# mokemokechicken/reversi-alpha-zero

Hardware: NVIDIA H100
Metric: self_play_games_per_sec (higher is better)
Workload: dtype f16

## Files before the change

reversi-alpha-zero_b200/csrc/rz_net_tc.cu:

```cuda
#include <stdlib.h>
#include <type_traits>
#include "rz_bitboard.cuh"
#include "rz_net.cuh"
#include "rz_tc_common.cuh"

namespace rz {
namespace tc {

constexpr uint32_t kProducerRegs = 40, kMathRegs = 232;
constexpr int kMathThreads = 256;
constexpr uint32_t kActCg = 2896, kActSlot = 144;
constexpr uint32_t kActBytes = 32 * kActCg;
constexpr uint32_t kStageBytes = 32768, kStages = 3;
constexpr int kResAhead = 4;
constexpr uint32_t kA0Bytes = 8192, kW0Bytes = 16384;
constexpr uint32_t kOffAct = 0;
constexpr uint32_t kOffW = kOffAct + kActBytes;
constexpr uint32_t kOffA0 = kOffW + kStages * kStageBytes;
constexpr uint32_t kOffW0 = kOffA0 + kA0Bytes;
constexpr uint32_t kOffSS = kOffW0 + kW0Bytes;
constexpr uint32_t kOffHw = kOffSS + 2 * 2048;
constexpr uint32_t kOffBar = kOffHw + 768 * 4;
constexpr uint32_t kNumBars = 2 * kStages + 1;
constexpr uint32_t kSmemBytes = kOffBar + kNumBars * 8;
constexpr uint32_t kSmemAlloc = kSmemBytes + 128;
static_assert(kSmemAlloc <= 232448, "shared memory budget exceeded");
static_assert(kTowerResFloatsPerCta == (size_t)kMathThreads * 128, "residual scratch per CTA");

#ifdef RZ_TOWER_STAMPS
enum : int {
    kStTiles,
    kStTile,
    kStKLoop,
    kStFull,
    kStMma,
    kStEpiBar,
    kStEpi0,
    kStEpi1,
    kStEpi2,
    kStEpiLast,
    kStFeat,
    kStEmpty,
    kStCount
};
constexpr int kStMaxCtas = 1024;
__device__ unsigned long long g_tower_stamps[kStMaxCtas][kStCount];
__device__ __forceinline__ void stamp_add(int phase, uint32_t cycles) { atomicAdd(&g_tower_stamps[blockIdx.x][phase], (unsigned long long)cycles); }
#define RZ_STAMP(...) __VA_ARGS__
#else
#define RZ_STAMP(...)
#endif

template <int CL>
__global__ void __launch_bounds__(kThreads, 1) net_tower_kernel(const Params pp) {
    Params p = pp;
    if (p.n_dev) p.n = *p.n_dev;
    extern __shared__ uint8_t smem_raw[];
    const uint32_t base = (smem_u32(smem_raw) + 127u) & ~127u;
    uint8_t* sm = smem_raw + (base - smem_u32(smem_raw));
    const int warp = threadIdx.x >> 5, lane = threadIdx.x & 31;
    const uint32_t bar0 = base + kOffBar;
    auto bar_full = [&](uint32_t s) { return bar0 + s * 8; };
    auto bar_empty = [&](uint32_t s) { return bar0 + (kStages + s) * 8; };
    const uint32_t bar_w0 = bar0 + 2 * kStages * 8;
    const uint32_t ntiles = (p.n + 1) >> 1;
    const int L = p.n_layers;
    const uint32_t crank = CL > 1 ? cluster_ctarank() : 0u;
    const uint32_t cbase = blockIdx.x - crank;
    const uint32_t iters = cbase < ntiles ? (ntiles - cbase + gridDim.x - 1) / gridDim.x : 0u;

    for (uint32_t i = threadIdx.x * 16; i < kActBytes; i += kThreads * 16) *reinterpret_cast<uint4*>(sm + kOffAct + i) = make_uint4(0, 0, 0, 0);
    fence_proxy_async();
    for (uint32_t i = threadIdx.x; i < 768; i += kThreads)
        reinterpret_cast<float*>(sm + kOffHw)[i] = __ldg(i < 512 ? p.blob + p.off_policy_conv + i : p.blob + p.off_value_conv + (i - 512));
    if (threadIdx.x == 0) {
        for (uint32_t s = 0; s < kStages; ++s) { mbar_init(bar_full(s), 1); mbar_init(bar_empty(s), 8 * CL); }
        mbar_init(bar_w0, 1);
        asm volatile("fence.mbarrier_init.release.cluster;" ::: "memory");
    }
    __syncthreads();
    if (CL > 1) cluster_sync_all();

    if (warp >= 8) {
        asm volatile("setmaxnreg.dec.sync.aligned.u32 %0;" ::"n"(kProducerRegs));
        if (warp == 8 && lane == 0) {
            if (iters > 0) {
                mbar_expect_tx(bar_w0, kW0Bytes);
                bulk_g2s(base + kOffW0, p.w0, kW0Bytes, bar_w0);
            }
            uint32_t stage = 0, phase = 0;
            for (uint32_t it = 0; it < iters; ++it) {
                for (int l = 1; l < L; ++l) {
                    const uint8_t* src = reinterpret_cast<const uint8_t*>(p.w) + (size_t)(l - 1) * 36 * kStageBytes;
                    RZ_STAMP(uint32_t st_empty = 0;)
                    for (int s = 0; s < 36; ++s) {
                        RZ_STAMP(const uint32_t c0 = (uint32_t)clock();)
                        mbar_wait(bar_empty(stage), phase ^ 1);
                        RZ_STAMP(st_empty += (uint32_t)clock() - c0;)
                        mbar_expect_tx(bar_full(stage), kStageBytes);
                        if (CL == 1) {
                            bulk_g2s(base + kOffW + stage * kStageBytes, src + (size_t)s * kStageBytes, kStageBytes, bar_full(stage));
                        } else {
                            constexpr uint32_t kSlice = kStageBytes / CL;
                            bulk_g2s_mc(base + kOffW + stage * kStageBytes + crank * kSlice, src + (size_t)s * kStageBytes + crank * kSlice,
                                        kSlice, bar_full(stage), (uint16_t)((1u << CL) - 1u));
                        }
                        if (++stage == kStages) { stage = 0; phase ^= 1; }
                    }
                    RZ_STAMP(stamp_add(kStEmpty, st_empty);)
                }
            }
        }
    } else {
        asm volatile("setmaxnreg.inc.sync.aligned.u32 %0;" ::"n"(kMathRegs));
        const int et = threadIdx.x;
        const int wg = warp >> 2;
        const int r0 = wg * 64 + (warp & 3) * 16 + (lane >> 2);
        const int g0 = r0 >> 3, x = r0 & 7, y = g0 >> 1;
        const int cq = 2 * (lane & 3);
        const uint32_t act_row0 = base + kOffAct + (g0 + 2) * kActSlot + (x + 1) * 16 + cq * 2;
        const uint32_t act_row1 = act_row0 + kActSlot;
        const uint32_t a_wg = base + kOffAct + wg * 8 * kActSlot;
        float* ss_s = reinterpret_cast<float*>(sm + kOffSS);
        float4* res = reinterpret_cast<float4*>(p.res + (size_t)blockIdx.x * kTowerResFloatsPerCta) + et;
        const float* hw = reinterpret_cast<const float*>(sm + kOffHw);
        uint32_t stage = 0, phase = 0, ss_buf = 0;
        float d[128];
        ss_s[et] = __ldg(p.ss + et);
        ss_s[256 + et] = __ldg(p.ss + 256 + et);

        for (uint32_t it = 0; it < iters; ++it) {
            const uint32_t tile = blockIdx.x + it * gridDim.x;
            const uint32_t pos0 = tile * 2;
            RZ_STAMP(const uint32_t st_tile0 = (uint32_t)clock();)
            {
                const int m = et & 127, g = m >> 3, brd = g & 1;
                const bool valid = pos0 + brd < p.n;
                build_layer0_operand(sm + kOffA0, valid ? p.own[pos0 + brd] : 0, valid ? p.enemy[pos0 + brd] : 0, 2 * (et >> 7), g, m & 7,
                                     g >> 1);
                fence_proxy_async();
            }
            float hs[6];
            for (int l = 0; l < L; ++l) {
                const float* sc = ss_s + ss_buf * 512;
                const bool is_conv2 = l > 0 && (l & 1) == 0;
                float4 rb[kResAhead];
                RZ_STAMP(uint32_t st_c = (uint32_t)clock(), st_bar = 0, st_full = 0, st_mma = 0;)
                epi_bar();
                RZ_STAMP(st_bar += (uint32_t)clock() - st_c;)
                {
                    const size_t nl = l + 1 < L ? (size_t)l + 1 : 0;
                    const uint32_t dst = smem_u32(ss_s + (ss_buf ^ 1) * 512 + et);
                    cp_async_4(dst, p.ss + nl * 512 + et);
                    cp_async_4(dst + 1024, p.ss + nl * 512 + 256 + et);
                }
                RZ_STAMP(const uint32_t st_k0 = (uint32_t)clock();)
                acc_fence(d);
                if (l == 0) {
                    RZ_STAMP(st_c = (uint32_t)clock();)
                    mbar_wait(bar_w0, 0);
                    RZ_STAMP(st_full += (uint32_t)clock() - st_c;)
                    wgmma_fence();
#pragma unroll
                    for (uint32_t j = 0; j < 2; ++j)
                        wgmma_m64n256k16(d, smem_desc(base + kOffA0 + j * 2 * 2048 + wg * 1024, 2048, 128),
                                         smem_desc(base + kOffW0 + j * 2 * 4096, 4096, 128), j);
                    wgmma_commit();
                    RZ_STAMP(st_c = (uint32_t)clock();)
                    wgmma_wait<0>();
                    RZ_STAMP(st_mma += (uint32_t)clock() - st_c;)
                } else {
                    int prev = -1;
                    for (uint32_t tap = 0; tap < 9; ++tap) {
                        const uint32_t a_tap = a_wg + (2 * (tap / 3)) * kActSlot + (tap % 3) * 16;
                        for (uint32_t kb = 0; kb < 4; ++kb) {
                            RZ_STAMP(st_c = (uint32_t)clock();)
                            mbar_wait(bar_full(stage), phase);
                            RZ_STAMP(st_full += (uint32_t)clock() - st_c;)
                            const uint32_t b_st = base + kOffW + stage * kStageBytes;
                            wgmma_fence();
#pragma unroll
                            for (uint32_t j = 0; j < 4; ++j)
                                wgmma_m64n256k16(d, smem_desc(a_tap + (kb * 8 + 2 * j) * kActCg, kActCg, kActSlot),
                                                 smem_desc(b_st + 2 * j * 4096, 4096, 128), (tap | kb | j) != 0);
                            wgmma_commit();
                            RZ_STAMP(st_c = (uint32_t)clock();)
                            wgmma_wait<1>();
                            RZ_STAMP(st_mma += (uint32_t)clock() - st_c;)
                            if (prev >= 0 && lane == 0) {
                                mbar_arrive(bar_empty(prev));
                                if (CL > 1) mbar_arrive_cta(bar_empty(prev), crank ^ 1u);
                            }
                            prev = (int)stage;
                            if (++stage == kStages) { stage = 0; phase ^= 1; }
                        }
                    }
                    if (is_conv2) {
#pragma unroll
                        for (int i = 0; i < kResAhead; ++i) rb[i] = res[i * 256];
                    }
                    RZ_STAMP(st_c = (uint32_t)clock();)
                    wgmma_wait<0>();
                    RZ_STAMP(st_mma += (uint32_t)clock() - st_c;)
                    if (lane == 0) {
                        mbar_arrive(bar_empty(prev));
                        if (CL > 1) mbar_arrive_cta(bar_empty(prev), crank ^ 1u);
                    }
                }
                RZ_STAMP(const uint32_t st_k1 = (uint32_t)clock();)
                acc_fence(d);
                cp_async_wait_all();
                ss_buf ^= 1;
                const bool keep_res = l == 0 || is_conv2;
                const bool last = l == L - 1;
                RZ_STAMP(st_c = (uint32_t)clock();)
                if (!last) epi_bar();
                RZ_STAMP(const uint32_t st_e0 = (uint32_t)clock(); st_bar += st_e0 - st_c;)
                float* dbg0 = nullptr;
                float* dbg1 = nullptr;
                if (last && p.dbg_tower) {
                    if (pos0 < p.n) dbg0 = p.dbg_tower + ((size_t)pos0 * 64 + y * 8 + x) * 256;
                    if (pos0 + 1 < p.n) dbg1 = p.dbg_tower + ((size_t)(pos0 + 1) * 64 + y * 8 + x) * 256;
                }
                constexpr int kEpiRelu = 0, kEpiKeep = 1, kEpiLast = 2;
                auto epilogue = [&](auto conv2, auto kind) {
                    constexpr bool kConv2 = decltype(conv2)::value;
                    constexpr bool kKeep = decltype(kind)::value == kEpiKeep, kLast = decltype(kind)::value == kEpiLast;
                    if (kLast) {
#pragma unroll
                        for (int k = 0; k < 6; ++k) hs[k] = 0.f;
                    }
#pragma unroll
                for (int i = 0; i < 32; ++i) {
                    const int c = 8 * i + cq;
                    const float2 s = *reinterpret_cast<const float2*>(sc + c);
                    const float2 b = *reinterpret_cast<const float2*>(sc + 256 + c);
                    float v0 = fmaf(d[4 * i + 0], s.x, b.x), v1 = fmaf(d[4 * i + 1], s.y, b.y);
                    float v2 = fmaf(d[4 * i + 2], s.x, b.x), v3 = fmaf(d[4 * i + 3], s.y, b.y);
                    if (kConv2) {
                        const float4 r = rb[i % kResAhead];
                        if (i + kResAhead < 32) rb[i % kResAhead] = res[(i + kResAhead) * 256];
                        v0 += r.x; v1 += r.y; v2 += r.z; v3 += r.w;
                    }
                    if (kKeep || kLast) {
                        v0 = fmaxf(v0, 0.f); v1 = fmaxf(v1, 0.f); v2 = fmaxf(v2, 0.f); v3 = fmaxf(v3, 0.f);
                    }
                    if (!kLast) {
                        if (kKeep) res[i * 256] = make_float4(v0, v1, v2, v3);
                        const uint32_t h0 = pack_h2<!kKeep>(v0, v1);
                        const uint32_t h1 = pack_h2<!kKeep>(v2, v3);
                        const uint32_t off = (c >> 3) * kActCg;
                        asm volatile("st.shared.b32 [%0], %1;" ::"r"(act_row0 + off), "r"(h0) : "memory");
                        asm volatile("st.shared.b32 [%0], %1;" ::"r"(act_row1 + off), "r"(h1) : "memory");
                    } else {
                        const float4 w = *reinterpret_cast<const float4*>(hw + 2 * c);
                        const float2 wv = *reinterpret_cast<const float2*>(hw + 512 + c);
                        hs[0] = fmaf(v1, w.z, fmaf(v0, w.x, hs[0]));
                        hs[1] = fmaf(v1, w.w, fmaf(v0, w.y, hs[1]));
                        hs[2] = fmaf(v1, wv.y, fmaf(v0, wv.x, hs[2]));
                        hs[3] = fmaf(v3, w.z, fmaf(v2, w.x, hs[3]));
                        hs[4] = fmaf(v3, w.w, fmaf(v2, w.y, hs[4]));
                        hs[5] = fmaf(v3, wv.y, fmaf(v2, wv.x, hs[5]));
                        if (dbg0) *reinterpret_cast<float2*>(dbg0 + c) = make_float2(v0, v1);
                        if (dbg1) *reinterpret_cast<float2*>(dbg1 + c) = make_float2(v2, v3);
                    }
                }
                };
                using Conv2 = std::true_type;
                using NoConv2 = std::false_type;
                if (last) {
                    if (is_conv2) epilogue(Conv2(), std::integral_constant<int, kEpiLast>());
                    else epilogue(NoConv2(), std::integral_constant<int, kEpiLast>());
                } else if (is_conv2) {
                    epilogue(Conv2(), std::integral_constant<int, kEpiKeep>());
                } else if (keep_res) {
                    epilogue(NoConv2(), std::integral_constant<int, kEpiKeep>());
                } else {
                    epilogue(NoConv2(), std::integral_constant<int, kEpiRelu>());
                }
                if (!last) fence_proxy_async();
                RZ_STAMP(if (et == 0) {
                    stamp_add(kStKLoop, st_k1 - st_k0); stamp_add(kStFull, st_full); stamp_add(kStMma, st_mma); stamp_add(kStEpiBar, st_bar);
                    stamp_add(l == 0 ? kStEpi0 : last ? kStEpiLast : is_conv2 ? kStEpi2 : kStEpi1, (uint32_t)clock() - st_e0);
                })
            }
            RZ_STAMP(const uint32_t st_h0 = (uint32_t)clock();)
#pragma unroll
            for (int k = 0; k < 6; ++k) {
                hs[k] += __shfl_xor_sync(0xffffffffu, hs[k], 1);
                hs[k] += __shfl_xor_sync(0xffffffffu, hs[k], 2);
            }
            {
                const int q = lane & 3;
                if (q < 2 && pos0 + q < p.n) {
                    const float h0 = q ? hs[3] : hs[0], h1 = q ? hs[4] : hs[1], h2 = q ? hs[5] : hs[2];
                    store_head_features(p.feat + (size_t)(pos0 + q) * kHeadFeatures, p.ss + (size_t)L * 512, y * 8 + x, h0 + 0.f,
                                        h1 + 0.f, h2 + 0.f);
                }
            }
            RZ_STAMP(if (et == 0) {
                const uint32_t st_h1 = (uint32_t)clock();
                stamp_add(kStFeat, st_h1 - st_h0); stamp_add(kStTile, st_h1 - st_tile0); stamp_add(kStTiles, 1);
            })
        }
    }

    __syncthreads();
    if (CL > 1) cluster_sync_all();
}

int launch_tower(const Params& p, cudaStream_t stream) {
    return launch_tower_pairs<net_tower_kernel<1>, net_tower_kernel<2>, kSmemAlloc, 2>(p, stream);
}

}

static int g_cluster = 0;

int set_tower_cluster(int cluster) {
    RZ_REQUIRE(cluster == 1 || cluster == 2, "rz_net_set_tower_cluster: cluster must be 1 or 2");
    g_cluster = cluster;
    return RZ_OK;
}

int tower_cluster() {
    if (g_cluster == 0) {
        const char* cs = getenv("RZ_TOWER_CLUSTER");
        g_cluster = (cs && atoi(cs) == 1) ? 1 : 2;
    }
    return g_cluster;
}

}

#ifdef RZ_TOWER_STAMPS
extern "C" int rz_tower_stamps(unsigned long long* out, int n_ctas, int reset) {
    using namespace rz::tc;
    if (n_ctas < 0 || n_ctas > kStMaxCtas) return (int)cudaErrorInvalidValue;
    const size_t bytes = (size_t)n_ctas * kStCount * sizeof(unsigned long long);
    cudaError_t e = cudaDeviceSynchronize();
    if (e == cudaSuccess && out) e = cudaMemcpyFromSymbol(out, g_tower_stamps, bytes);
    if (e == cudaSuccess && reset) {
        void* dev = nullptr;
        e = cudaGetSymbolAddress(&dev, g_tower_stamps);
        if (e == cudaSuccess) e = cudaMemset(dev, 0, sizeof(g_tower_stamps));
        if (e == cudaSuccess) e = cudaDeviceSynchronize();
    }
    return (int)e;
}
extern "C" int rz_tower_stamp_count() { return rz::tc::kStCount; }
#endif
```

reversi-alpha-zero_b200/csrc/rz_tc_common.cuh:

```cuda
#pragma once
#include <cuda_fp16.h>
#include "rz_bitboard.cuh"
#include "rz_net.cuh"

namespace rz {
namespace tc {

__device__ __forceinline__ uint32_t smem_u32(const void* p) { return (uint32_t)__cvta_generic_to_shared(p); }

__device__ __forceinline__ void mbar_init(uint32_t bar, uint32_t count) {
    asm volatile("mbarrier.init.shared::cta.b64 [%0], %1;" ::"r"(bar), "r"(count) : "memory");
}
__device__ __forceinline__ void mbar_expect_tx(uint32_t bar, uint32_t bytes) {
    asm volatile("mbarrier.arrive.expect_tx.shared::cta.b64 _, [%0], %1;" ::"r"(bar), "r"(bytes) : "memory");
}
__device__ __forceinline__ void mbar_arrive(uint32_t bar) {
    asm volatile("mbarrier.arrive.shared::cta.b64 _, [%0];" ::"r"(bar) : "memory");
}
__device__ __forceinline__ void mbar_arrive_cta(uint32_t bar, uint32_t rank) {
    uint32_t remote;
    asm volatile("mapa.shared::cluster.u32 %0, %1, %2;" : "=r"(remote) : "r"(bar), "r"(rank));
    asm volatile("mbarrier.arrive.shared::cluster.b64 _, [%0];" ::"r"(remote) : "memory");
}
__device__ __forceinline__ void mbar_wait(uint32_t bar, uint32_t parity) {
    uint32_t ok = 0;
    long long t0 = 0;
    for (uint32_t spin = 0; !ok; ++spin) {
        asm volatile(
            "{\n\t.reg .pred p;\n\t"
            "mbarrier.try_wait.parity.shared::cta.b64 p, [%1], %2;\n\t"
            "selp.u32 %0, 1, 0, p;\n\t}"
            : "=r"(ok)
            : "r"(bar), "r"(parity)
            : "memory");
        if (!ok && (spin & 1023) == 1023) {
            const long long now = clock64();
            if (t0 == 0) t0 = now;
            else if (now - t0 > 8000000000LL) __trap();
        }
    }
}
__device__ __forceinline__ void bulk_g2s(uint32_t dst, const void* src, uint32_t bytes, uint32_t bar) {
    asm volatile("cp.async.bulk.shared::cluster.global.mbarrier::complete_tx::bytes [%0], [%1], %2, [%3];" ::"r"(dst), "l"(src),
                 "r"(bytes), "r"(bar)
                 : "memory");
}
__device__ __forceinline__ void bulk_g2s_mc(uint32_t dst, const void* src, uint32_t bytes, uint32_t bar, uint16_t mask) {
    asm volatile(
        "cp.async.bulk.shared::cluster.global.mbarrier::complete_tx::bytes.multicast::cluster [%0], [%1], %2, [%3], %4;" ::"r"(dst),
        "l"(src), "r"(bytes), "r"(bar), "h"(mask)
        : "memory");
}
__device__ __forceinline__ void cluster_sync_all() {
    asm volatile("barrier.cluster.arrive.release.aligned;\n\tbarrier.cluster.wait.acquire.aligned;" ::: "memory");
}
__device__ __forceinline__ uint32_t cluster_ctarank() {
    uint32_t r;
    asm volatile("mov.u32 %0, %%cluster_ctarank;" : "=r"(r));
    return r;
}
__device__ __forceinline__ void cp_async_4(uint32_t dst, const void* src) {
    asm volatile("cp.async.ca.shared.global [%0], [%1], 4;" ::"r"(dst), "l"(src) : "memory");
}
__device__ __forceinline__ void cp_async_wait_all() { asm volatile("cp.async.wait_all;" ::: "memory"); }
__device__ __forceinline__ void fence_proxy_async() { asm volatile("fence.proxy.async.shared::cta;" ::: "memory"); }
__device__ __forceinline__ void epi_bar() { asm volatile("bar.sync 1, 256;" ::: "memory"); }

__device__ __forceinline__ uint64_t smem_desc(uint32_t addr, uint32_t lbo, uint32_t sbo) {
    return (uint64_t)((addr >> 4) & 0x3FFF) | ((uint64_t)((lbo >> 4) & 0x3FFF) << 16) | ((uint64_t)((sbo >> 4) & 0x3FFF) << 32);
}
__device__ __forceinline__ void wgmma_fence() { asm volatile("wgmma.fence.sync.aligned;" ::: "memory"); }
__device__ __forceinline__ void wgmma_commit() { asm volatile("wgmma.commit_group.sync.aligned;" ::: "memory"); }
template <int N>
__device__ __forceinline__ void wgmma_wait() { asm volatile("wgmma.wait_group.sync.aligned %0;" ::"n"(N) : "memory"); }
__device__ __forceinline__ void acc_fence(float (&d)[128]) {
#pragma unroll
    for (int i = 0; i < 128; ++i) asm volatile("" : "+f"(d[i])::"memory");
}

#define RZ_D4(i) "+f"(d[i]), "+f"(d[i + 1]), "+f"(d[i + 2]), "+f"(d[i + 3])
#define RZ_D16(i) RZ_D4(i), RZ_D4(i + 4), RZ_D4(i + 8), RZ_D4(i + 12)
__device__ __forceinline__ void wgmma_m64n256k16(float (&d)[128], uint64_t adesc, uint64_t bdesc, uint32_t accumulate) {
    asm volatile(
        "{\n\t.reg .pred p;\n\t"
        "setp.ne.b32 p, %130, 0;\n\t"
        "wgmma.mma_async.sync.aligned.m64n256k16.f32.f16.f16 {"
        "%0, %1, %2, %3, %4, %5, %6, %7, %8, %9, %10, %11, %12, %13, %14, %15, "
        "%16, %17, %18, %19, %20, %21, %22, %23, %24, %25, %26, %27, %28, %29, %30, %31, "
        "%32, %33, %34, %35, %36, %37, %38, %39, %40, %41, %42, %43, %44, %45, %46, %47, "
        "%48, %49, %50, %51, %52, %53, %54, %55, %56, %57, %58, %59, %60, %61, %62, %63, "
        "%64, %65, %66, %67, %68, %69, %70, %71, %72, %73, %74, %75, %76, %77, %78, %79, "
        "%80, %81, %82, %83, %84, %85, %86, %87, %88, %89, %90, %91, %92, %93, %94, %95, "
        "%96, %97, %98, %99, %100, %101, %102, %103, %104, %105, %106, %107, %108, %109, %110, %111, "
        "%112, %113, %114, %115, %116, %117, %118, %119, %120, %121, %122, %123, %124, %125, %126, %127"
        "}, %128, %129, p, 1, 1, 0, 0;\n\t}"
        : RZ_D16(0), RZ_D16(16), RZ_D16(32), RZ_D16(48), RZ_D16(64), RZ_D16(80), RZ_D16(96), RZ_D16(112)
        : "l"(adesc), "l"(bdesc), "r"(accumulate)
        : "memory");
}
template <int O>
__device__ __forceinline__ void wgmma_m64n128k16(float (&d)[128], uint64_t adesc, uint64_t bdesc, uint32_t accumulate) {
    asm volatile(
        "{\n\t.reg .pred p;\n\t"
        "setp.ne.b32 p, %66, 0;\n\t"
        "wgmma.mma_async.sync.aligned.m64n128k16.f32.f16.f16 {"
        "%0, %1, %2, %3, %4, %5, %6, %7, %8, %9, %10, %11, %12, %13, %14, %15, "
        "%16, %17, %18, %19, %20, %21, %22, %23, %24, %25, %26, %27, %28, %29, %30, %31, "
        "%32, %33, %34, %35, %36, %37, %38, %39, %40, %41, %42, %43, %44, %45, %46, %47, "
        "%48, %49, %50, %51, %52, %53, %54, %55, %56, %57, %58, %59, %60, %61, %62, %63"
        "}, %64, %65, p, 1, 1, 0, 0;\n\t}"
        : RZ_D16(O), RZ_D16(O + 16), RZ_D16(O + 32), RZ_D16(O + 48)
        : "l"(adesc), "l"(bdesc), "r"(accumulate)
        : "memory");
}
template <int O>
__device__ __forceinline__ void wgmma_m64n64k16(float (&d)[128], uint64_t adesc, uint64_t bdesc, uint32_t accumulate) {
    asm volatile(
        "{\n\t.reg .pred p;\n\t"
        "setp.ne.b32 p, %34, 0;\n\t"
        "wgmma.mma_async.sync.aligned.m64n64k16.f32.f16.f16 {"
        "%0, %1, %2, %3, %4, %5, %6, %7, %8, %9, %10, %11, %12, %13, %14, %15, "
        "%16, %17, %18, %19, %20, %21, %22, %23, %24, %25, %26, %27, %28, %29, %30, %31"
        "}, %32, %33, p, 1, 1, 0, 0;\n\t}"
        : RZ_D16(O), RZ_D16(O + 16)
        : "l"(adesc), "l"(bdesc), "r"(accumulate)
        : "memory");
}
#undef RZ_D16
#undef RZ_D4

template <bool RELU>
__device__ __forceinline__ uint32_t pack_h2(float a, float b) {
    uint32_t d;
    if (RELU) asm("cvt.rn.relu.satfinite.f16x2.f32 %0, %1, %2;" : "=r"(d) : "f"(b), "f"(a));
    else      asm("cvt.rn.satfinite.f16x2.f32 %0, %1, %2;" : "=r"(d) : "f"(b), "f"(a));
    return d;
}

struct Params {
    const __half* w0;
    const __half* w;
    const float* ss;
    const float* blob;
    size_t off_policy_conv, off_policy_fc_k, off_policy_fc_b, off_value_conv, off_value_fc1_k, off_value_fc1_b, off_value_fc2_k,
        off_value_fc2_b;
    const u64* own;
    const u64* enemy;
    float* policy;
    float* value;
    float* res;
    float* feat;
    float* dbg_tower;
    float* dbg_logits;
    float* dbg_vlogit;
    uint32_t n;
    const uint32_t* n_dev;
    int n_layers;
    int V;
};

constexpr uint32_t kTcMaxV = 512;

constexpr int kThreads = 384;

template <void (*K1)(Params), void (*K2)(Params), uint32_t kSmem, uint32_t kBoards>
int launch_tower_pairs(const Params& p, cudaStream_t stream) {
    static int max_pairs = -1;
    if (max_pairs < 0) {
        RZ_CUDA_TRY(cudaFuncSetAttribute(K1, cudaFuncAttributeMaxDynamicSharedMemorySize, (int)kSmem));
        RZ_CUDA_TRY(cudaFuncSetAttribute(K2, cudaFuncAttributeMaxDynamicSharedMemorySize, (int)kSmem));
        cudaLaunchConfig_t cfg = {};
        cfg.gridDim = dim3((unsigned)num_sms() & ~1u); cfg.blockDim = dim3(kThreads); cfg.dynamicSmemBytes = kSmem;
        cudaLaunchAttribute attr[1];
        attr[0].id = cudaLaunchAttributeClusterDimension;
        attr[0].val.clusterDim.x = 2; attr[0].val.clusterDim.y = 1; attr[0].val.clusterDim.z = 1;
        cfg.attrs = attr; cfg.numAttrs = 1;
        RZ_CUDA_TRY(cudaOccupancyMaxActiveClusters(&max_pairs, K2, &cfg));
    }
    const int cluster = tower_cluster() == 2 && max_pairs >= 1 ? 2 : 1;
    const uint32_t ntiles = (p.n + kBoards - 1) / kBoards;
    uint32_t grid = ntiles < (uint32_t)num_sms() ? ntiles : (uint32_t)num_sms();
    if (cluster == 1) {
        K1<<<grid, kThreads, kSmem, stream>>>(p);
    } else {
        grid = (grid + 1) & ~1u;
        if (grid > 2u * (uint32_t)max_pairs) grid = 2u * (uint32_t)max_pairs;
        cudaLaunchConfig_t cfg = {};
        cfg.gridDim = dim3(grid); cfg.blockDim = dim3(kThreads); cfg.dynamicSmemBytes = kSmem; cfg.stream = stream;
        cudaLaunchAttribute attr[1];
        attr[0].id = cudaLaunchAttributeClusterDimension;
        attr[0].val.clusterDim.x = 2; attr[0].val.clusterDim.y = 1; attr[0].val.clusterDim.z = 1;
        cfg.attrs = attr; cfg.numAttrs = 1;
        RZ_CUDA_TRY(cudaLaunchKernelEx(&cfg, K2, p));
    }
    RZ_LAUNCH_CHECK();
    return RZ_OK;
}

int launch_tower(const Params& p, cudaStream_t stream);
int launch_tower_narrow(const Params& p, int filters, cudaStream_t stream);
int launch_tower_split(const Params& p, cudaStream_t stream);

__device__ __forceinline__ void build_layer0_operand(uint8_t* a0, u64 o, u64 e, int kc0, int g, int x, int y) {
#pragma unroll
    for (int kk = 0; kk < 2; ++kk) {
        const int kc = kc0 + kk;
        uint32_t w[4];
#pragma unroll
        for (int jp = 0; jp < 4; ++jp) {
            uint32_t packed = 0;
#pragma unroll
            for (int half = 0; half < 2; ++half) {
                const int k = kc * 8 + jp * 2 + half;
                uint32_t bit = 0;
                if (k < 18) {
                    const int tap = k >> 1, yy = y + tap / 3 - 1, xx = x + tap % 3 - 1;
                    if (yy >= 0 && yy < 8 && xx >= 0 && xx < 8) bit = (uint32_t)((((k & 1) ? e : o) >> (yy * 8 + xx)) & 1ULL);
                }
                packed |= (bit ? 0x3C00u : 0u) << (16 * half);
            }
            w[jp] = packed;
        }
        *reinterpret_cast<uint4*>(a0 + kc * 2048 + g * 128 + x * 16) = make_uint4(w[0], w[1], w[2], w[3]);
    }
}

__device__ __forceinline__ void store_head_features(float* f, const float* ssh, int pix, float a0, float a1, float av) {
    f[pix] = fmaxf(fmaf(a0, ssh[0], ssh[2]), 0.f);
    f[64 + pix] = fmaxf(fmaf(a1, ssh[1], ssh[3]), 0.f);
    f[128 + pix] = fmaxf(fmaf(av, ssh[4], ssh[5]), 0.f);
}

}

int net_heads(const tc::Params& p, cudaStream_t stream);

}
```

Before: 24.29.

## Transpose tower GEMM so weights are A operand and activations B, skip padded tap columns

The conv GEMM is reformulated so that weights (channels) form the M dimension and board positions form N, using m64n128/m64n112 wgmma instead of m64n256 with activations as A. The 9 taps are regrouped by kernel row into 36 stages, and the last kernel row issues narrower n112 MMAs to skip padding columns. The epilogue now writes activations back with stmatrix transposes, and the head-feature reduction stages fp32 values through shared memory with extra barriers. This restructures operand layout and data reuse in exchange for more complex indexing and an additional shared-memory pass in the final layer.

After: 24.74 (median of 6 runs). +1.9%, better.

```diff
diff --git a/reversi-alpha-zero_b200/csrc/rz_net_tc.cu b/reversi-alpha-zero_b200/csrc/rz_net_tc.cu
--- a/reversi-alpha-zero_b200/csrc/rz_net_tc.cu
+++ b/reversi-alpha-zero_b200/csrc/rz_net_tc.cu
@@ -3,6 +3,7 @@
 #include "rz_bitboard.cuh"
 #include "rz_net.cuh"
 #include "rz_tc_common.cuh"
+#include "rz_tower_cols.cuh"
 
 namespace rz {
 namespace tc {
@@ -50,6 +51,29 @@
 #else
 #define RZ_STAMP(...)
 #endif
+
+template <int O, int C0, int N>
+__device__ __forceinline__ void wgmma_cols(float (&d)[128], uint32_t a, uint32_t b, uint32_t accumulate) {
+    const uint64_t adesc = smem_desc(a, 4096, 128), bdesc = smem_desc(b + C0 / 8 * kActSlot, kActCg, kActSlot);
+    if constexpr (N == 128) wgmma_m64n128k16<O + tap_reg0(TapCols{C0, N})>(d, adesc, bdesc, accumulate);
+    else wgmma_m64n112k16<O + tap_reg0(TapCols{C0, N})>(d, adesc, bdesc, accumulate);
+}
+
+template <int KH, bool FIRST>
+__device__ __forceinline__ void conv_stage(float (&d)[128], uint32_t a_st, uint32_t b_k) {
+    constexpr TapCols f = tap_cols(KH, FIRST), t = tap_cols(KH, false);
+#pragma unroll
+    for (uint32_t j = 0; j < 4; ++j) {
+        const uint32_t a = a_st + 2 * j * 4096, b = b_k + 2 * j * kActCg;
+        if (FIRST && j == 0) {
+            wgmma_cols<0, f.col0, f.ncols>(d, a, b, 0);
+            wgmma_cols<64, f.col0, f.ncols>(d, a + 1024, b, 0);
+        } else {
+            wgmma_cols<0, t.col0, t.ncols>(d, a, b, 1);
+            wgmma_cols<64, t.col0, t.ncols>(d, a + 1024, b, 1);
+        }
+    }
+}
 
 template <int CL>
 __global__ void __launch_bounds__(kThreads, 1) net_tower_kernel(const Params pp) {
@@ -115,12 +139,11 @@
         asm volatile("setmaxnreg.inc.sync.aligned.u32 %0;" ::"n"(kMathRegs));
         const int et = threadIdx.x;
         const int wg = warp >> 2;
-        const int r0 = wg * 64 + (warp & 3) * 16 + (lane >> 2);
-        const int g0 = r0 >> 3, x = r0 & 7, y = g0 >> 1;
-        const int cq = 2 * (lane & 3);
-        const uint32_t act_row0 = base + kOffAct + (g0 + 2) * kActSlot + (x + 1) * 16 + cq * 2;
-        const uint32_t act_row1 = act_row0 + kActSlot;
-        const uint32_t a_wg = base + kOffAct + wg * 8 * kActSlot;
+        const int chq = 128 * wg + 16 * (warp & 3) + (lane >> 2);
+        const int q = lane & 3;
+        const uint32_t w_wg = 2 * wg * 1024;
+        const uint32_t st_row = base + kOffAct + (uint32_t)((chq >> 3) + ((lane >> 3) & 1)) * kActCg + ((lane >> 4) + 2) * kActSlot +
+                                ((lane & 7) + 1) * 16;
         float* ss_s = reinterpret_cast<float*>(sm + kOffSS);
         float4* res = reinterpret_cast<float4*>(p.res + (size_t)blockIdx.x * kTowerResFloatsPerCta) + et;
         const float* hw = reinterpret_cast<const float*>(sm + kOffHw);
@@ -140,7 +163,6 @@
                                      g >> 1);
                 fence_proxy_async();
             }
-            float hs[6];
             for (int l = 0; l < L; ++l) {
                 const float* sc = ss_s + ss_buf * 512;
                 const bool is_conv2 = l > 0 && (l & 1) == 0;
@@ -162,39 +184,43 @@
                     RZ_STAMP(st_full += (uint32_t)clock() - st_c;)
                     wgmma_fence();
 #pragma unroll
-                    for (uint32_t j = 0; j < 2; ++j)
-                        wgmma_m64n256k16(d, smem_desc(base + kOffA0 + j * 2 * 2048 + wg * 1024, 2048, 128),
-                                         smem_desc(base + kOffW0 + j * 2 * 4096, 4096, 128), j);
+                    for (uint32_t j = 0; j < 2; ++j) {
+                        const uint32_t a = base + kOffW0 + j * 2 * 4096 + w_wg;
+                        const uint64_t b = smem_desc(base + kOffA0 + j * 2 * 2048, 2048, 128);
+                        wgmma_m64n128k16<0>(d, smem_desc(a, 4096, 128), b, j);
+                        wgmma_m64n128k16<64>(d, smem_desc(a + 1024, 4096, 128), b, j);
+                    }
                     wgmma_commit();
                     RZ_STAMP(st_c = (uint32_t)clock();)
                     wgmma_wait<0>();
                     RZ_STAMP(st_mma += (uint32_t)clock() - st_c;)
                 } else {
                     int prev = -1;
-                    for (uint32_t tap = 0; tap < 9; ++tap) {
-                        const uint32_t a_tap = a_wg + (2 * (tap / 3)) * kActSlot + (tap % 3) * 16;
-                        for (uint32_t kb = 0; kb < 4; ++kb) {
-                            RZ_STAMP(st_c = (uint32_t)clock();)
-                            mbar_wait(bar_full(stage), phase);
-                            RZ_STAMP(st_full += (uint32_t)clock() - st_c;)
-                            const uint32_t b_st = base + kOffW + stage * kStageBytes;
-                            wgmma_fence();
-#pragma unroll
-                            for (uint32_t j = 0; j < 4; ++j)
-                                wgmma_m64n256k16(d, smem_desc(a_tap + (kb * 8 + 2 * j) * kActCg, kActCg, kActSlot),
-                                                 smem_desc(b_st + 2 * j * 4096, 4096, 128), (tap | kb | j) != 0);
-                            wgmma_commit();
-                            RZ_STAMP(st_c = (uint32_t)clock();)
-                            wgmma_wait<1>();
-                            RZ_STAMP(st_mma += (uint32_t)clock() - st_c;)
-                            if (prev >= 0 && lane == 0) {
-                                mbar_arrive(bar_empty(prev));
-                                if (CL > 1) mbar_arrive_cta(bar_empty(prev), crank ^ 1u);
-                            }
-                            prev = (int)stage;
-                            if (++stage == kStages) { stage = 0; phase ^= 1; }
+                    auto run_stage = [&](auto kh_c, auto first_c, uint32_t s) {
+                        constexpr int KH = decltype(kh_c)::value;
+                        const uint32_t b_k = base + kOffAct + 2 * KH * kActSlot + (s >> 2) * 16 + (s & 3) * 8 * kActCg;
+                        RZ_STAMP(st_c = (uint32_t)clock();)
+                        mbar_wait(bar_full(stage), phase);
+                        RZ_STAMP(st_full += (uint32_t)clock() - st_c;)
+                        wgmma_fence();
+                        conv_stage<KH, decltype(first_c)::value>(d, base + kOffW + stage * kStageBytes + w_wg, b_k);
+                        wgmma_commit();
+                        RZ_STAMP(st_c = (uint32_t)clock();)
+                        wgmma_wait<1>();
+                        RZ_STAMP(st_mma += (uint32_t)clock() - st_c;)
+                        if (prev >= 0 && lane == 0) {
+                            mbar_arrive(bar_empty(prev));
+                            if (CL > 1) mbar_arrive_cta(bar_empty(prev), crank ^ 1u);
                         }
-                    }
+                        prev = (int)stage;
+                        if (++stage == kStages) { stage = 0; phase ^= 1; }
+                    };
+                    using First = std::true_type;
+                    using NotFirst = std::false_type;
+                    run_stage(std::integral_constant<int, 0>(), First(), 0);
+                    for (uint32_t s = 1; s < 12; ++s) run_stage(std::integral_constant<int, 0>(), NotFirst(), s);
+                    for (uint32_t s = 0; s < 12; ++s) run_stage(std::integral_constant<int, 1>(), NotFirst(), s);
+                    for (uint32_t s = 0; s < 12; ++s) run_stage(std::integral_constant<int, 2>(), NotFirst(), s);
                     if (is_conv2) {
 #pragma unroll
                         for (int i = 0; i < kResAhead; ++i) rb[i] = res[i * 256];
@@ -216,54 +242,47 @@
                 RZ_STAMP(st_c = (uint32_t)clock();)
                 if (!last) epi_bar();
                 RZ_STAMP(const uint32_t st_e0 = (uint32_t)clock(); st_bar += st_e0 - st_c;)
-                float* dbg0 = nullptr;
-                float* dbg1 = nullptr;
-                if (last && p.dbg_tower) {
-                    if (pos0 < p.n) dbg0 = p.dbg_tower + ((size_t)pos0 * 64 + y * 8 + x) * 256;
-                    if (pos0 + 1 < p.n) dbg1 = p.dbg_tower + ((size_t)(pos0 + 1) * 64 + y * 8 + x) * 256;
-                }
                 constexpr int kEpiRelu = 0, kEpiKeep = 1, kEpiLast = 2;
                 auto epilogue = [&](auto conv2, auto kind) {
                     constexpr bool kConv2 = decltype(conv2)::value;
                     constexpr bool kKeep = decltype(kind)::value == kEpiKeep, kLast = decltype(kind)::value == kEpiLast;
-                    if (kLast) {
-#pragma unroll
-                        for (int k = 0; k < 6; ++k) hs[k] = 0.f;
-                    }
-#pragma unroll
-                for (int i = 0; i < 32; ++i) {
-                    const int c = 8 * i + cq;
-                    const float2 s = *reinterpret_cast<const float2*>(sc + c);
-                    const float2 b = *reinterpret_cast<const float2*>(sc + 256 + c);
-                    float v0 = fmaf(d[4 * i + 0], s.x, b.x), v1 = fmaf(d[4 * i + 1], s.y, b.y);
-                    float v2 = fmaf(d[4 * i + 2], s.x, b.x), v3 = fmaf(d[4 * i + 3], s.y, b.y);
-                    if (kConv2) {
-                        const float4 r = rb[i % kResAhead];
-                        if (i + kResAhead < 32) rb[i % kResAhead] = res[(i + kResAhead) * 256];
-                        v0 += r.x; v1 += r.y; v2 += r.z; v3 += r.w;
-                    }
-                    if (kKeep || kLast) {
-                        v0 = fmaxf(v0, 0.f); v1 = fmaxf(v1, 0.f); v2 = fmaxf(v2, 0.f); v3 = fmaxf(v3, 0.f);
-                    }
-                    if (!kLast) {
-                        if (kKeep) res[i * 256] = make_float4(v0, v1, v2, v3);
-                        const uint32_t h0 = pack_h2<!kKeep>(v0, v1);
-                        const uint32_t h1 = pack_h2<!kKeep>(v2, v3);
-                        const uint32_t off = (c >> 3) * kActCg;
-                        asm volatile("st.shared.b32 [%0], %1;" ::"r"(act_row0 + off), "r"(h0) : "memory");
-                        asm volatile("st.shared.b32 [%0], %1;" ::"r"(act_row1 + off), "r"(h1) : "memory");
-                    } else {
-                        const float4 w = *reinterpret_cast<const float4*>(hw + 2 * c);
-                        const float2 wv = *reinterpret_cast<const float2*>(hw + 512 + c);
-                        hs[0] = fmaf(v1, w.z, fmaf(v0, w.x, hs[0]));
-                        hs[1] = fmaf(v1, w.w, fmaf(v0, w.y, hs[1]));
-                        hs[2] = fmaf(v1, wv.y, fmaf(v0, wv.x, hs[2]));
-                        hs[3] = fmaf(v3, w.z, fmaf(v2, w.x, hs[3]));
-                        hs[4] = fmaf(v3, w.w, fmaf(v2, w.y, hs[4]));
-                        hs[5] = fmaf(v3, wv.y, fmaf(v2, wv.x, hs[5]));
-                        if (dbg0) *reinterpret_cast<float2*>(dbg0 + c) = make_float2(v0, v1);
-                        if (dbg1) *reinterpret_cast<float2*>(dbg1 + c) = make_float2(v2, v3);
-                    }
+                    float s[4], b[4];
+#pragma unroll
+                    for (int k = 0; k < 4; ++k) {
+                        const int ch = chq + 64 * (k >> 1) + 8 * (k & 1);
+                        s[k] = sc[ch];
+                        b[k] = sc[256 + ch];
+                    }
+#pragma unroll
+                for (int i = 0; i < 32; i += 2) {
+                    uint32_t h[4];
+#pragma unroll
+                    for (int u = 0; u < 2; ++u) {
+                        const int k = i + u, kb = 2 * (k >> 4);
+                        float v0 = fmaf(d[4 * k + 0], s[kb], b[kb]), v1 = fmaf(d[4 * k + 1], s[kb], b[kb]);
+                        float v2 = fmaf(d[4 * k + 2], s[kb + 1], b[kb + 1]), v3 = fmaf(d[4 * k + 3], s[kb + 1], b[kb + 1]);
+                        if (kConv2) {
+                            const float4 r = rb[k % kResAhead];
+                            if (k + kResAhead < 32) rb[k % kResAhead] = res[(k + kResAhead) * 256];
+                            v0 += r.x; v1 += r.y; v2 += r.z; v3 += r.w;
+                        }
+                        if (kKeep || kLast) {
+                            v0 = fmaxf(v0, 0.f); v1 = fmaxf(v1, 0.f); v2 = fmaxf(v2, 0.f); v3 = fmaxf(v3, 0.f);
+                        }
+                        if (!kLast) {
+                            if (kKeep) res[k * 256] = make_float4(v0, v1, v2, v3);
+                            h[2 * u] = pack_h2<!kKeep>(v0, v1);
+                            h[2 * u + 1] = pack_h2<!kKeep>(v2, v3);
+                        } else {
+                            d[4 * k + 0] = v0; d[4 * k + 1] = v1; d[4 * k + 2] = v2; d[4 * k + 3] = v3;
+                            const int g = k & 15;
+                            if (p.dbg_tower && pos0 + (g & 1) < p.n) {
+                                float* t = p.dbg_tower + ((size_t)(pos0 + (g & 1)) * 64 + (g >> 1) * 8 + 2 * q) * 256 + chq + 64 * (k >> 4);
+                                t[0] = v0; t[256] = v1; t[8] = v2; t[264] = v3;
+                            }
+                        }
+                    }
+                    if (!kLast) stmatrix_x4_trans(st_row + (i >> 4) * 8 * kActCg + (i & 15) * kActSlot, h[0], h[1], h[2], h[3]);
                 }
                 };
                 using Conv2 = std::true_type;
@@ -285,17 +304,47 @@
                 })
             }
             RZ_STAMP(const uint32_t st_h0 = (uint32_t)clock();)
-#pragma unroll
-            for (int k = 0; k < 6; ++k) {
-                hs[k] += __shfl_xor_sync(0xffffffffu, hs[k], 1);
-                hs[k] += __shfl_xor_sync(0xffffffffu, hs[k], 2);
-            }
+            epi_bar();
             {
-                const int q = lane & 3;
-                if (q < 2 && pos0 + q < p.n) {
-                    const float h0 = q ? hs[3] : hs[0], h1 = q ? hs[4] : hs[1], h2 = q ? hs[5] : hs[2];
-                    store_head_features(p.feat + (size_t)(pos0 + q) * kHeadFeatures, p.ss + (size_t)L * 512, y * 8 + x, h0 + 0.f,
-                                        h1 + 0.f, h2 + 0.f);
+                const int e = lane >> 4;
+                const uint32_t st_w = kOffAct + (uint32_t)(chq >> 3) * kActCg + (2 + 8 * e) * kActSlot + ((lane >> 2) & 3) * 4;
+                const uint32_t ld_x = lane >> 2, ld_e = q >> 1;
+                const uint32_t ld = kOffAct + (2 + warp + 8 * ld_e) * kActSlot + ((ld_x ^ ld_e) + 1) * 16 + 8 * (q & 1);
+#pragma unroll
+                for (int hh = 0; hh < 2; ++hh) {
+                    if (hh) epi_bar();
+#pragma unroll
+                    for (int k = 0; k < 32; ++k) {
+                        const int g = (k & 15) - 8 * hh;
+                        if (g < 0 || g >= 8) continue;
+                        const uint32_t at = st_w + (uint32_t)(8 * (k >> 4)) * kActCg + g * kActSlot;
+#pragma unroll
+                        for (int r = 0; r < 4; ++r)
+                            *reinterpret_cast<float*>(sm + at + (r >> 1) * kActCg + (((2 * q + (r & 1)) ^ e) + 1) * 16) = d[4 * k + r];
+                    }
+                    epi_bar();
+                    float h0 = 0.f, h1 = 0.f, h2 = 0.f;
+#pragma unroll 8
+                    for (int i = 0; i < 32; ++i) {
+                        const int c = 8 * i + 2 * q;
+                        const float2 v = *reinterpret_cast<const float2*>(sm + ld + i * kActCg);
+                        const float4 w = *reinterpret_cast<const float4*>(hw + 2 * c);
+                        const float2 wv = *reinterpret_cast<const float2*>(hw + 512 + c);
+                        h0 = fmaf(v.y, w.z, fmaf(v.x, w.x, h0));
+                        h1 = fmaf(v.y, w.w, fmaf(v.x, w.y, h1));
+                        h2 = fmaf(v.y, wv.y, fmaf(v.x, wv.x, h2));
+                    }
+                    h0 += __shfl_xor_sync(0xffffffffu, h0, 1);
+                    h1 += __shfl_xor_sync(0xffffffffu, h1, 1);
+                    h2 += __shfl_xor_sync(0xffffffffu, h2, 1);
+                    h0 += __shfl_xor_sync(0xffffffffu, h0, 2);
+                    h1 += __shfl_xor_sync(0xffffffffu, h1, 2);
+                    h2 += __shfl_xor_sync(0xffffffffu, h2, 2);
+                    const int g = 8 * hh + warp, brd = g & 1;
+                    if (q == 0 && pos0 + brd < p.n) {
+                        store_head_features(p.feat + (size_t)(pos0 + brd) * kHeadFeatures, p.ss + (size_t)L * 512, (g >> 1) * 8 + ld_x,
+                                            h0 + 0.f, h1 + 0.f, h2 + 0.f);
+                    }
                 }
             }
             RZ_STAMP(if (et == 0) {
diff --git a/reversi-alpha-zero_b200/csrc/rz_tc_common.cuh b/reversi-alpha-zero_b200/csrc/rz_tc_common.cuh
--- a/reversi-alpha-zero_b200/csrc/rz_tc_common.cuh
+++ b/reversi-alpha-zero_b200/csrc/rz_tc_common.cuh
@@ -80,24 +80,6 @@
 
 #define RZ_D4(i) "+f"(d[i]), "+f"(d[i + 1]), "+f"(d[i + 2]), "+f"(d[i + 3])
 #define RZ_D16(i) RZ_D4(i), RZ_D4(i + 4), RZ_D4(i + 8), RZ_D4(i + 12)
-__device__ __forceinline__ void wgmma_m64n256k16(float (&d)[128], uint64_t adesc, uint64_t bdesc, uint32_t accumulate) {
-    asm volatile(
-        "{\n\t.reg .pred p;\n\t"
-        "setp.ne.b32 p, %130, 0;\n\t"
-        "wgmma.mma_async.sync.aligned.m64n256k16.f32.f16.f16 {"
-        "%0, %1, %2, %3, %4, %5, %6, %7, %8, %9, %10, %11, %12, %13, %14, %15, "
-        "%16, %17, %18, %19, %20, %21, %22, %23, %24, %25, %26, %27, %28, %29, %30, %31, "
-        "%32, %33, %34, %35, %36, %37, %38, %39, %40, %41, %42, %43, %44, %45, %46, %47, "
-        "%48, %49, %50, %51, %52, %53, %54, %55, %56, %57, %58, %59, %60, %61, %62, %63, "
-        "%64, %65, %66, %67, %68, %69, %70, %71, %72, %73, %74, %75, %76, %77, %78, %79, "
-        "%80, %81, %82, %83, %84, %85, %86, %87, %88, %89, %90, %91, %92, %93, %94, %95, "
-        "%96, %97, %98, %99, %100, %101, %102, %103, %104, %105, %106, %107, %108, %109, %110, %111, "
-        "%112, %113, %114, %115, %116, %117, %118, %119, %120, %121, %122, %123, %124, %125, %126, %127"
-        "}, %128, %129, p, 1, 1, 0, 0;\n\t}"
-        : RZ_D16(0), RZ_D16(16), RZ_D16(32), RZ_D16(48), RZ_D16(64), RZ_D16(80), RZ_D16(96), RZ_D16(112)
-        : "l"(adesc), "l"(bdesc), "r"(accumulate)
-        : "memory");
-}
 template <int O>
 __device__ __forceinline__ void wgmma_m64n128k16(float (&d)[128], uint64_t adesc, uint64_t bdesc, uint32_t accumulate) {
     asm volatile(
@@ -126,8 +108,29 @@
         : "l"(adesc), "l"(bdesc), "r"(accumulate)
         : "memory");
 }
+template <int O>
+__device__ __forceinline__ void wgmma_m64n112k16(float (&d)[128], uint64_t adesc, uint64_t bdesc, uint32_t accumulate) {
+    asm volatile(
+        "{\n\t.reg .pred p;\n\t"
+        "setp.ne.b32 p, %58, 0;\n\t"
+        "wgmma.mma_async.sync.aligned.m64n112k16.f32.f16.f16 {"
+        "%0, %1, %2, %3, %4, %5, %6, %7, %8, %9, %10, %11, %12, %13, %14, %15, "
+        "%16, %17, %18, %19, %20, %21, %22, %23, %24, %25, %26, %27, %28, %29, %30, %31, "
+        "%32, %33, %34, %35, %36, %37, %38, %39, %40, %41, %42, %43, %44, %45, %46, %47, "
+        "%48, %49, %50, %51, %52, %53, %54, %55"
+        "}, %56, %57, p, 1, 1, 0, 0;\n\t}"
+        : RZ_D16(O), RZ_D16(O + 16), RZ_D16(O + 32), RZ_D4(O + 48), RZ_D4(O + 52)
+        : "l"(adesc), "l"(bdesc), "r"(accumulate)
+        : "memory");
+}
 #undef RZ_D16
 #undef RZ_D4
+
+__device__ __forceinline__ void stmatrix_x4_trans(uint32_t addr, uint32_t r0, uint32_t r1, uint32_t r2, uint32_t r3) {
+    asm volatile("stmatrix.sync.aligned.m8n8.x4.trans.shared.b16 [%0], {%1, %2, %3, %4};" ::"r"(addr), "r"(r0), "r"(r1), "r"(r2),
+                 "r"(r3)
+                 : "memory");
+}
 
 template <bool RELU>
 __device__ __forceinline__ uint32_t pack_h2(float a, float b) {
diff --git a/reversi-alpha-zero_b200/csrc/rz_tower_cols.cuh b/reversi-alpha-zero_b200/csrc/rz_tower_cols.cuh
--- /dev/null
+++ b/reversi-alpha-zero_b200/csrc/rz_tower_cols.cuh
@@ -0,0 +1,18 @@
+#pragma once
+
+namespace rz {
+namespace tc {
+
+struct TapCols {
+    int col0;
+    int ncols;
+};
+
+constexpr TapCols tap_cols(int kh, bool first) {
+    return kh == 2 && !first ? TapCols{0, 112} : TapCols{0, 128};
+}
+
+constexpr int tap_reg0(TapCols t) { return t.col0 / 2; }
+
+}
+}
```
